# hadleyhzy34/porl

Hardware: AMD Instinct MI355X
Metric: gradient-steps/sec (POR update, batch=1024) (higher is better)
Workload: dtype f32; 1 GPU; POR S=60 A=2 H=1024 L=2 B=1024/GPU (global 1024), 1000000 -row replay (1000000/GPU) resident in HBM, device sampler + gather + full update per step; parallelism=dp1, global_batch=1024

## Files before the change

porl_amd/agent/_iql.py:

```python
from __future__ import annotations

import math
import warnings

import torch
import torch.nn as nn

from ..engine import IqlEngine
from ..parallel import GradExchange



_PIPE_SYNC = __import__("os").environ.get("PORL_PIPE_SYNC", "signal2")
_PIPE_ONECALL = __import__("os").environ.get("PORL_PIPE_ONECALL", "auto")
_DP_POLICY_GROUP = __import__("os").environ.get("PORL_DP_POLICY_GROUP", "1") != "0"
_ONECALL_MAX_WORK = 32 << 20

class ArenaAdam:

    def __init__(self, agent, group, named_params, lr):
        self._agent, self._group = agent, group
        self._names = [n for n, _ in named_params]
        self._params = [p for _, p in named_params]
        self.step_count = 0
# ... 178 lines not shown
                                     wait_policy_seq=max(0, seq - eng.SLOTS) if _PIPE_SYNC == "signal" else 0,
                                     wait_fwd_seq=vr[1] if isinstance(vr, tuple) else 0,
                                     write_policy=_PIPE_SYNC == "signal")
            except Exception:
                eng._seq -= 1
                v_opt.step_count -= 1
                p_opt.step_count -= 1
                raise
            replay.draws += 1
            eng._values_read, eng._policy_done = ("sig", seq), True
            sched.step()
            return self._losses()
        if use_sig:
            main = torch.cuda.current_stream(eng.device)
            eng._seq += 1
            seq = eng._seq
            if _PIPE_SYNC == "signal":
                eng.wait_signal(eng.SIG_POLICY, seq - eng.SLOTS, main)
        elif pipelined:
            eng.wait_slot_free()
        if replay is not None:
            B = eng.load_batch_sampled(replay.rows, batch, replay.seed, replay.draws, replay.act_dim,
                                       self._engine.cfg.weight_mode == 1)
            replay.draws += 1
        else:
            B = eng.load_batch(obs, next_obs, rew, term, pol_target)
        v_opt.step_count += 1
        p_opt.step_count += 1
        hp = self._hyper(B, v_opt, p_opt)
        if not dp and not pipelined:
            eng.step(hp)
            sched.step()
            return self._losses()
        eng.value_backward(hp)
        if dp and self._sharded():
            self._sharded_apply(IqlEngine.GROUP_VF, hp, v_opt)
        else:
            if dp:
                v_opt._unshard()
                ex.allreduce_sum_(eng.grads_vf)
            eng.wait_values_read()
            eng.value_apply(hp)
        if pipelined:
            main, side = torch.cuda.current_stream(eng.device), eng.side_stream()
            k = (v_opt.step_count % eng.SLOTS) * 3
            ev_v, ev_f, ev_p = eng.event(k), eng.event(k + 1), eng.event(k + 2)
            if use_sig:
                eng.signal(eng.SIG_VALUE, seq, main)
            else:
                ev_v.record(main)
            with torch.cuda.stream(side):
                if use_sig:
                    eng.wait_signal(eng.SIG_VALUE, seq, side)
                else:
                    side.wait_event(ev_v)
                eng.policy_forward(hp)
                if use_sig:
                    eng.signal(eng.SIG_FWD, seq, side)
                else:
                    ev_f.record(side)
                eng.policy_backward(hp)
                if dp and self._sharded():
                    self._sharded_apply(IqlEngine.GROUP_POL, hp, p_opt, self._exchange_for(IqlEngine.GROUP_POL, True))
                else:
                    if dp:
                        p_opt._unshard()
# ... 149 lines not shown
```

porl_amd/csrc/porl_api.hip:

```cpp
#include <hip/hip_runtime.h>

#include <algorithm>
#include <cmath>
#include <cstdio>
#include <cstring>
#include <string>
#include <vector>

#include "../../include/porl_hip.h"
#include "gemm_f32.hpp"
#include "gemm_bf16.hpp"
#include "kernels.hpp"
#include "l0_fwd.hpp"
#include "skinny.hpp"
#include "iqn.hpp"
#include "qnet_fused.hpp"
#include "per_tree.hpp"
#include "dist_losses.hpp"
#include "online.hpp"
#include "per_online.hpp"
#include "bcq_mask.hpp"

using namespace porl;

namespace {

thread_local std::string g_err;

#define PORL_FAIL(code, ...)                         \
  do {                                               \
    char _b[512];                                    \
    snprintf(_b, sizeof _b, __VA_ARGS__);            \
    g_err = _b;                                      \
    return (code);                                   \
  } while (0)
// ... 48 lines not shown
} g_prof;

const char* g_phase = "";

struct ProfScope {
  bool active; ProfRec r; hipStream_t s;
  ProfScope(const std::string& label, hipStream_t st, double flops, double bytes) : active(g_prof.on), s(st) {
    if (!active) return;
    r.label = g_prof.label_id(std::string(g_phase) + label); r.flops = flops; r.bytes = bytes;
    r.e0 = g_prof.get(); r.e1 = g_prof.get();
    (void)hipEventRecord(r.e0, s);
  }
  ~ProfScope() {
    if (!active) return;
    (void)hipEventRecord(r.e1, s);
    g_prof.recs.push_back(r);
  }
};

const float* g_dbg_a_scale = nullptr; const float* g_dbg_a_shift = nullptr; const float* g_dbg_resid = nullptr;
float* g_dbg_cstat = nullptr;
unsigned long long* g_qnet_stamps = nullptr;

constexpr int NUM_CU = 256;
constexpr int SK_MAX = 16;
constexpr int NLL_ROWS_PER_BLOCK = 4;
constexpr int LN_ROWS_PER_BLOCK = 8;
constexpr int HEAD_ROWS_PER_BLOCK = HEAD_ROWS;

struct Tune {
  int tile_map[4] = {TILE_64x128, TILE_64x64, TILE_64x128, TILE_64x64};
  int tile_map_short[4] = {TILE_64x64, TILE_64x64, TILE_64x128, TILE_64x64};
  int vbwd_tile_short = -1;
  int l0_kernel = 1;
  int l0_tile = -1;
  int skinny = 7;
  int skinny_pipelined = -1, skinny_pipelined_max_h = 768;
  int dw0_slabs = 16;
  int iql_fold = 1;
  int gemm_lds_pad = 0, gemm_lds_pad_min_blocks = 0;
  int iql_pad_value = 18432, iql_pad_policy = 0, iql_pad_min_blocks = 4 * NUM_CU, iql_pad_min_k = 0;
  int enc_tile_n96 = 0;
  int enc_gemm_sb = 1;
  int enc_patch_rows = 0;
  int enc_s2d = 0;
  int enc_bf16_operands_only = 0;
  int enc_pconv_mfma = 0;
  int enc_bn_sweep = 0;
  int enc_dense_patch = 0;
  int qnet_fused = 1;
  int qnet_rows16 = 1;
  int qnet_wgrad_share = 11;
  int qnet_two_groups = 1;
} g_tune;

enum TuneClamp { TC_ANY, TC_BOOL, TC_NONNEG, TC_1_16, TC_MASK };
struct TuneKey { const char* key; int Tune::*field; TuneClamp clamp; };
#define TK(key, clamp) {#key, &Tune::key, clamp}
const TuneKey k_tune_keys[] = {
    TK(gemm_lds_pad, TC_NONNEG), TK(gemm_lds_pad_min_blocks, TC_NONNEG), TK(iql_pad_value, TC_NONNEG), TK(iql_pad_policy, TC_NONNEG),
    TK(iql_pad_min_blocks, TC_NONNEG), TK(iql_pad_min_k, TC_NONNEG), TK(qnet_fused, TC_BOOL), TK(qnet_two_groups, TC_BOOL),
    TK(qnet_wgrad_share, TC_1_16), TK(qnet_rows16, TC_BOOL), TK(enc_dense_patch, TC_BOOL), TK(enc_s2d, TC_BOOL), TK(enc_patch_rows, TC_NONNEG),
    TK(enc_gemm_sb, TC_ANY), TK(enc_tile_n96, TC_BOOL), TK(enc_bn_sweep, TC_BOOL), TK(enc_pconv_mfma, TC_BOOL), TK(enc_bf16_operands_only, TC_BOOL),
    TK(iql_fold, TC_BOOL), TK(skinny, TC_MASK), TK(skinny_pipelined, TC_MASK), TK(skinny_pipelined_max_h, TC_ANY), TK(dw0_slabs, TC_1_16),
    TK(l0_tile, TC_ANY), TK(l0_kernel, TC_BOOL), TK(vbwd_tile_short, TC_ANY),
};

int tune_apply(Tune& t, const char* key, int value) {
  if (!key) PORL_FAIL(PORL_ERR_INVALID, "null key");
  for (const TuneKey& k : k_tune_keys) {
    if (strcmp(key, k.key)) continue;
    const TuneClamp c = k.clamp;
    t.*k.field = c == TC_BOOL ? value != 0 : c == TC_NONNEG ? std::max(0, value) : c == TC_1_16 ? std::max(1, std::min(value, 16))
               : c == TC_MASK && value == 1 ? 7 : value;
    return PORL_OK;
  }
  const bool sh = !strncmp(key, "tile_map_short", 14);
  const char* i = key + (sh ? 14 : 8);
  if (!strncmp(key, "tile_map", 8) && *i >= '0' && *i <= '3' && !i[1] && value >= 0 && value < TILE_COUNT) {
    (sh ? t.tile_map_short : t.tile_map)[*i - '0'] = value;
    return PORL_OK;
  }
  PORL_FAIL(PORL_ERR_INVALID, "unknown tuning key '%s'", key);
}

inline int64_t ru4(int64_t x) { return (x + 3) & ~int64_t(3); }
inline int cdiv(int a, int b) { return (a + b - 1) / b; }

struct TensorInfo { int64_t off; int rows, cols; };

struct MlpLayout {
  int n_lin = 0;
  int dims[PORL_MAX_HIDDEN + 2] = {0};
  int64_t w[PORL_MAX_HIDDEN + 1] = {0}, b[PORL_MAX_HIDDEN + 1] = {0};
  int64_t lnw[PORL_MAX_HIDDEN] = {0}, lnb[PORL_MAX_HIDDEN] = {0};
  bool ln = false;
};

// ... 28 lines not shown
  int64_t hp_t[2], hp_v[2];
  int64_t act_q[2][2], hp_q[2];
  int64_t dv[2], dmu;
  int64_t slab_mean, slab_a, slab_b, slab_pa;
  int64_t part_loss, part_min, part_dls;
  int64_t xhat_v[2][PORL_MAX_HIDDEN], rstd_v[2][PORL_MAX_HIDDEN];
  int64_t ln_dg[2], ln_db[2], ln_dh[2];
  int64_t head_part[2], head_loss, head_db[2];
  int64_t pol_w;
  int64_t total;
};

}

struct porl_iql {
  porl_iql_cfg cfg;
  MlpLayout v[2], pol;
  int64_t logstd_off = 0, n_vf = 0, n_pol = 0;
  std::vector<TensorInfo> t_vf, t_pol;
  porl_iql_buffers buf{};
  bool bound = false;
  int device = -1;
  int mode = 0;
  int slot = 0;
  ReduceArgs fin_v{}, fin_p{};
  bool fin_v_pending = false, fin_p_pending = false;
  int batch = 0;
  bool have_pol_target = false;
  bool pol_prefetched = false;
  bool pol_fwd_done = false;
  int pol_nslab = 1;
  int Sp = 0, Dp = 0, Hp = 0, parts_max = 0;
  Workspace ws{};
  Tune tune = g_tune;
};

namespace {

int pick_tile(const GemmGroup& g, const Tune& t, bool short_blocks = false) {
  int minM = 1 << 30, minN = 1 << 30, maxK = 0;
  for (int i = 0; i < g.nprob; ++i) {
    minM = std::min(minM, g.p[i].M); minN = std::min(minN, g.p[i].N); maxK = std::max(maxK, g.p[i].K);
  }
  if (maxK <= 128) return TILE_64x64;
  auto blocks = [&](int tile) {
    int bm, bn, n = 0;
    tile_dims(tile, bm, bn);
    for (int i = 0; i < g.nprob; ++i) n += cdiv(g.p[i].M, bm) * cdiv(g.p[i].N, bn) * std::max(1, g.p[i].splitk);
    return n;
  };
  int cand[3], nc = 0;
  if (minN <= 64 && minM <= 64) { cand[nc++] = TILE_64x64; }
  else if (minN <= 64) { cand[nc++] = TILE_128x64; cand[nc++] = TILE_64x64; }
  else if (minM <= 64) { cand[nc++] = TILE_64x128; cand[nc++] = TILE_64x64; }
  else { cand[nc++] = TILE_128x128; cand[nc++] = TILE_128x64; cand[nc++] = TILE_64x64; }
  const int* map = short_blocks ? t.tile_map_short : t.tile_map;
  for (int i = 0; i < nc; ++i)
    if (blocks(cand[i]) >= NUM_CU) return map[cand[i]];
  return map[cand[nc - 1]];
}

int pick_splitk(int M, int N, int K, int nprob, int bm, int bn) {
  const int tiles = nprob * cdiv(M, bm) * cdiv(N, bn);
  int sk = cdiv(NUM_CU, tiles);
  sk = std::min(sk, std::max(1, K / 64));
  return std::max(1, std::min(sk, SK_MAX));
}

int launch_group(GemmGroup& g, int tile, const Tune& t, hipStream_t s, int iql_pad = -1) {
  const bool iql = iql_pad >= 0 && !t.gemm_lds_pad && g.nprob > 0 && g.p[0].K >= t.iql_pad_min_k;
  g.lds_pad = iql ? iql_pad : t.gemm_lds_pad;
  g.lds_pad_min_blocks = iql ? t.iql_pad_min_blocks : t.gemm_lds_pad_min_blocks;
  double flops = 0.0, bytes = 0.0;
  std::string label;
  if (g_prof.on) {
    bool vec = true, apro = false;
    for (int i = 0; i < g.nprob; ++i) {
      const GemmProb& p = g.p[i];
      flops += 2.0 * p.M * p.N * p.K;
      bytes += 4.0 * ((double)p.M * p.K + (double)p.N * p.K + (p.store_c ? (double)p.M * p.N : 0.0));
      vec = vec && p.a_vec && p.b_vec;
      apro = apro || p.apro != APRO_NONE;
    }
    int bm, bn;
    tile_dims(tile, bm, bn);
    const TileCfg tc = tile_cfg(tile);
    label = "gemm_f32_kernel<" + std::to_string(bm) + "," + std::to_string(bn) + "," + std::to_string(GEMM_BK) + "," +
            std::to_string(tc.wm) + "," + std::to_string(tc.wn) + "," + (vec ? "true" : "false") + "," +
            (apro ? "true" : "false") + (g.single_buffer && vec && tile == TILE_64x64 ? ",true>" : ">");
  }
  ProfScope ps(label, s, flops, bytes);
  hipError_t e = launch_gemm_group(tile, g, s);
  if (e != hipSuccess) {
    g_err = std::string("gemm launch: ") + hipGetErrorString(e);
    return (int)e;
  }
  return 0;
}

int launch_group_bf16(GemmGroup& g, int tile, hipStream_t s) {
  double flops = 0.0, bytes = 0.0;
  std::string label;
  if (g_prof.on) {
    for (int i = 0; i < g.nprob; ++i) {
      const GemmProb& p = g.p[i];
// ... 18 lines not shown
  if (r.njobs == 0) return 0;
  long maxn = 0;
  for (int i = 0; i < r.njobs; ++i) maxn = std::max(maxn, r.job[i].n);
  dim3 grid((unsigned)std::min<long>((maxn + 31) / 32, 2048), r.njobs);
  ProfScope ps("multi_reduce_kernel", s, 0.0, 0.0);
  hipLaunchKernelGGL(multi_reduce_kernel, grid, dim3(256), 0, s, r);
  PORL_HIP(hipGetLastError());
  return 0;
}

void add_reduce(ReduceArgs& r, float* out, const float* slab, long n, long stride, int nslab, int op = 0,
                float scale = 1.f) {
  ReduceJob& j = r.job[r.njobs++];
  j.out = out; j.slab = slab; j.bias = nullptr; j.n = n; j.stride = stride; j.nslab = nslab; j.ncols = 1; j.act = 0;
  j.op = op; j.scale = scale; j.adam_off = -1;
  j.width = nslab > 64 ? 4 : 32;
}

int check_ready(const porl_iql* h, bool need_batch) {
  if (!h) PORL_FAIL(PORL_ERR_INVALID, "null engine");
  if (!h->bound) PORL_FAIL(PORL_ERR_UNBOUND, "porl_iql_bind() has not been called");
  if (need_batch && h->batch <= 0) PORL_FAIL(PORL_ERR_INVALID, "no minibatch loaded (porl_iql_load_batch)");
  return 0;
}

bool short_blocks(const porl_iql* h) { return (h->mode & PORL_IQL_MODE_SHORT_BLOCKS) != 0; }
int skinny_mask(const porl_iql* h) {
  const Tune& t = h->tune;
  if (!short_blocks(h)) return t.skinny;
  return t.skinny_pipelined >= 0 ? t.skinny_pipelined : h->cfg.hidden_dim <= t.skinny_pipelined_max_h ? t.skinny : 0;
}
int iql_tile(const porl_iql* h, const GemmGroup& g) { return pick_tile(g, h->tune, short_blocks(h)); }

int iql_launch(const porl_iql* h, GemmGroup& g, int tile, bool policy, hipStream_t s) {
  const Tune& t = h->tune;
  return launch_group(g, tile, t, s, !short_blocks(h) ? -1 : policy ? t.iql_pad_policy : t.iql_pad_value);
}

constexpr int MAX_FWD_NETS = 5;
struct FwdNet {
  const float* in; int ldin;
  const float* W; const float* b;
  float* out;
  const float* headw; float* headout;
  const float* ln_g = nullptr; const float* ln_b = nullptr;
  float* xhat = nullptr; float* rstd = nullptr;
};

int fwd_hidden_layer(porl_iql* h, const FwdNet* nets, int nnets, int B, int K, bool last, int* parts_out, bool policy,
                     hipStream_t s) {
  const int H = h->cfg.hidden_dim;
  if (h->tune.l0_kernel && K <= L0_KP && nnets <= L0_MAX_NETS) {
    L0Args a{};
    a.nnets = nnets; a.B = B; a.H = H; a.K = K; a.ldw = K; a.ldo = h->Hp;
    bool plain = true;
    for (int n = 0; n < nnets; ++n) {
      plain = plain && !nets[n].ln_g && nets[n].out && !(last && nets[n].headw);
      a.net[n] = L0Net{nets[n].in, nets[n].W, nets[n].b, nets[n].out, nets[n].ldin};
    }
    if (plain && l0_fwd_supported(a)) {
      if (parts_out) *parts_out = head_parts(H, 0);
      ProfScope ps("l0_fwd_kernel", s, 2.0 * nnets * B * (double)H * K, 4.0 * nnets * ((double)B * K + (double)H * K + (double)B * H));
      PORL_HIP(launch_l0_fwd(a, s));
      return 0;
    }
  }
  GemmGroup g{};
  g.nprob = nnets;
  bool any_ln = false;
// ... 352 lines not shown
      a.hp_t[i] = W + ws.hp_t[i]; a.hp_v[i] = W + ws.hp_v[i];
      a.b_t[i] = Pt + h->v[i].b[L]; a.b_v[i] = Pv + h->v[i].b[L];
      a.dv[i] = W + ws.dv[i];
      a.db_out[i] = Gv + h->v[i].b[L];
    }
    a.rew = W + ws.rew; a.term = W + ws.term; a.target_v = W + ws.target_v_slot[h->slot]; a.stats = h->buf.stats;
    a.B = B; a.parts = parts; a.tau = hp->tau; a.discount = hp->discount; a.inv_batch = hp->inv_batch;
    hipLaunchKernelGGL(value_loss_kernel, dim3(1), dim3(1024), 0, s, a);
    PORL_HIP(hipGetLastError());
  }

  ReduceArgs red{};
  if (LN) return value_backward_ln(h, hp, s, defer);
  {
    const int nhb = cdiv(B, HEAD_ROWS_PER_BLOCK);
    HeadBwdArgs a{};
    for (int i = 0; i < 2; ++i) {
      a.Hact[i] = W + ws.act_v[i][L - 1]; a.w[i] = Pv + h->v[i].w[L];
      a.dZ[i] = W + ws.dz_v[i][(L - 1) & 1]; a.part_dw[i] = W + ws.head_part[i];
      a.hp_t[i] = W + ws.hp_t[i]; a.hp_v[i] = W + ws.hp_v[i];
      a.b_t[i] = Pt + h->v[i].b[L]; a.b_v[i] = Pv + h->v[i].b[L];
      a.dv[i] = W + ws.dv[i]; a.part_db[i] = W + ws.head_db[i];
      add_reduce(red, Gv + h->v[i].w[L], W + ws.head_part[i], H, H, nhb);
      add_reduce(red, Gv + h->v[i].b[L], W + ws.head_db[i], 1, 1, nhb);
    }
    a.rew = W + ws.rew; a.term = W + ws.term; a.target_v = W + ws.target_v_slot[h->slot]; a.part_loss = W + ws.head_loss;
    add_reduce(red, h->buf.stats, W + ws.head_loss, 1, 1, nhb, 0, hp->inv_batch);
    a.B = B; a.H = H; a.ld = Hp; a.parts = parts;
    a.tau = hp->tau; a.discount = hp->discount; a.inv_batch = hp->inv_batch;
    ProfScope ps("relu_head_bwd_kernel", s, 0.0, 16.0 * B * H);
    hipLaunchKernelGGL(relu_head_bwd_kernel, dim3(nhb, 2), dim3(256), 0, s, a);
    PORL_HIP(hipGetLastError());
  }
  for (int l = L - 1; l >= 0; --l) {
    const int Kin = l == 0 ? S : H;
    if (l == 0) {
      Dw0Net dn[2];
      const int64_t per = (int64_t)H * S, perc = H;
      for (int i = 0; i < 2; ++i) {
        float* slabW = W + ws.slab_a + (int64_t)i * SK_MAX * (per + 2 * perc + 8);
        dn[i] = Dw0Net{W + ws.dz_v[i][0], Gv + h->v[i].w[0], Gv + h->v[i].b[0], slabW, slabW + (int64_t)SK_MAX * per};
      }
      int rc = 0;
      if (dw0_skinny(h, dn, 2, W + ws.xs_slot[h->slot], h->Sp, B, H, S, Hp, red, "V6.dW0:", s, &rc)) {
        if (rc) return rc;
        break;
      }
    }
    GemmGroup g{};
    for (int i = 0; i < 2; ++i) {
      const float* dz = W + ws.dz_v[i][l & 1];
      const float* in = l == 0 ? W + ws.xs_slot[h->slot] : W + ws.act_v[i][l - 1];
      const int ldin = l == 0 ? h->Sp : Hp;
      GemmProb p = make_prob(GEMM_TN, dz, Hp, in, ldin, Gv + h->v[i].w[l], Kin, H, Kin, B);
      p.colsum = Gv + h->v[i].b[l];
      g.p[g.nprob++] = p;
      if (l > 0) {
        GemmProb q = make_prob(GEMM_NN, dz, Hp, Pv + h->v[i].w[l], Kin, W + ws.dz_v[i][(l - 1) & 1], Hp, B, Kin, H);
        q.mask = W + ws.act_v[i][l - 1]; q.ldmask = Hp;
        g.p[g.nprob++] = q;
      }
    }
    int tile = iql_tile(h, g);
    if (l > 0 && short_blocks(h) && h->tune.vbwd_tile_short >= 0) tile = h->tune.vbwd_tile_short;
    if (l == 0) {
      int bm, bn;
      tile_dims(tile, bm, bn);
      const int sk = pick_splitk(H, Kin, B, 2, bm, bn);
      if (sk > 1) {
        const int64_t per = (int64_t)H * Kin, perc = H;
        for (int i = 0; i < 2; ++i) {
          float* slabW = W + ws.slab_a + (int64_t)i * SK_MAX * (per + 2 * perc + 8);
          float* slabC = slabW + (int64_t)SK_MAX * per;
          g.p[i].splitk = sk; g.p[i].C = slabW; g.p[i].colsum = slabC;
          add_reduce(red, Gv + h->v[i].w[0], slabW, per, per, sk);
          add_reduce(red, Gv + h->v[i].b[0], slabC, perc, perc, sk);
        }
      }
    }
    g_phase = l == 0 ? "V6.dW0:" : "V5.bwd:";
    PORL_TRY(iql_launch(h, g, tile, false, s));
  }
  g_phase = "V7.combine:";
  if (defer) *defer = red;
  else PORL_TRY(launch_reduce(red, s));
  g_phase = "";
  return PORL_OK;
}

int porl_iql_value_backward(porl_iql* h, const porl_iql_hyper* hp, void* stream) {
  PORL_TRY(check_ready(h, true)); DevGuard _dg(h->device);
  if (!hp) PORL_FAIL(PORL_ERR_INVALID, "null hyper-parameters");
  const bool fold = (h->mode & PORL_IQL_MODE_FOLD_COMBINE) != 0;
  h->fin_v = ReduceArgs{};
  PORL_TRY(value_backward_impl(h, hp, (hipStream_t)stream, fold ? &h->fin_v : nullptr));
  h->fin_v_pending = fold;
  return PORL_OK;
}

static int adam_launch(float* p, float* g, float* m, float* v, float* tgt, int64_t n, double lr, int step,
                       double b1, double b2, double eps, double ema_beta, hipStream_t s, const ReduceArgs* fin = nullptr) {
  if (n < 0 || n % 4) PORL_FAIL(PORL_ERR_INVALID, "adam range must be a non-negative multiple of 4 floats");
  if (step < 1) PORL_FAIL(PORL_ERR_INVALID, "adam step must be >= 1");
  if (n == 0 && !(fin && fin->njobs)) return PORL_OK;
  AdamArgs a{};
  a.p = p; a.g = g; a.m = m; a.v = v; a.tgt = tgt;
  const double bc1 = 1.0 - std::pow(b1, (double)step);
  const double bc2 = 1.0 - std::pow(b2, (double)step);
  a.s.step_size = (float)(lr / bc1);
  a.s.bc2_sqrt = (float)std::sqrt(bc2);
  a.s.omb1 = (float)(1.0 - b1); a.s.beta2 = (float)b2; a.s.omb2 = (float)(1.0 - b2);
  a.s.eps = (float)eps; a.s.ema_beta = (float)ema_beta; a.s.omeb = (float)(1.0 - ema_beta);
  a.n4 = n / 4;
  const int sweep_blocks = (int)std::min<long>((a.n4 + 255) / 256, 1 << 20);
  a.span4 = sweep_blocks ? ((a.n4 + sweep_blocks - 1) / sweep_blocks + 255) / 256 * 256 : 256;
  int reduce_blocks = 0;
  double extra_bytes = 0.0;
  if (fin) {
    for (int q = 0; q < fin->njobs; ++q) {
      ReduceJob j = fin->job[q];
      const bool inside = j.out >= g && j.out + j.n <= g + n;
      const long off = inside ? (long)(j.out - g) : -1;
      extra_bytes += 4.0 * (double)j.n * j.nslab;
      const bool plain = j.op == 0 && j.scale == 1.f && !j.bias && j.act == 0;
      if (inside && plain && j.nslab <= ADAM_SWEEP_SLABS && off % 4 == 0 && j.n % 4 == 0 && j.stride % 4 == 0 &&
          aligned16(j.slab) && a.nregions < MAX_ADAM_REGIONS) {
        AdamRegion& R = a.region[a.nregions++];
        R.lo = off; R.hi = off + j.n; R.slab = j.slab; R.stride = j.stride; R.nslab = j.nslab;
// ... 220 lines not shown
    a.tiles_n = cdiv(H, SKN_T);
    skn_split(cdiv(B, SKN_T), SK_MAX, a.nslab, a.rtiles);
    a.slabW_stride = (long)D * H; a.slabC_stride = D;
    add_reduce(red, Gp + h->pol.w[L], a.slabW, (long)D * H, (long)D * H, a.nslab);
    add_reduce(red, Gp + h->pol.b[L], a.slabC, D, D, a.nslab);
    g_phase = "P5.outbwd:";
    {
      ProfScope ps("out_bwd_kernel", s, 4.0 * B * (double)H * D, 4.0 * (2.0 * B * H + (double)B * D + (double)D * H + (double)a.nslab * D * H));
      hipLaunchKernelGGL(out_bwd_kernel, dim3(a.nslab * a.tiles_n), dim3(256), 0, s, a);
    }
    g_phase = "";
    PORL_HIP(hipGetLastError());
  } else {
    GemmGroup g{};
    g.nprob = 2;
    g.p[0] = make_prob(GEMM_TN, W + ws.dmu, Dp, W + ws.act_p[L - 1], Hp, Gp + h->pol.w[L], H, D, H, B);
    g.p[0].colsum = Gp + h->pol.b[L];
    g.p[1] = make_prob(GEMM_NN, W + ws.dmu, Dp, Pp + h->pol.w[L], H, W + ws.dz_p[(L - 1) & 1], Hp, B, H, D);
    g.p[1].mask = W + ws.act_p[L - 1]; g.p[1].ldmask = Hp;
    const int tile = D <= 64 ? TILE_64x128 : iql_tile(h, g);
    int bm, bn;
    tile_dims(tile, bm, bn);
    const int sk = pick_splitk(D, H, B, 1, bm, bn);
    if (sk > 1) {
      float* slabW = W + ws.slab_b;
      float* slabC = slabW + (int64_t)SK_MAX * D * H;
      g.p[0].splitk = sk; g.p[0].C = slabW; g.p[0].colsum = slabC;
      add_reduce(red, Gp + h->pol.w[L], slabW, (long)D * H, (long)D * H, sk);
      add_reduce(red, Gp + h->pol.b[L], slabC, D, D, sk);
    }
    g_phase = "P5.outbwd:";
    PORL_TRY(iql_launch(h, g, tile, true, s));
  }
  for (int l = L - 1; l >= 0; --l) {
    const int Kin = l == 0 ? S : H;
    if (l == 0) {
      const int64_t per = (int64_t)H * S;
      float* slabW = W + ws.slab_pa;
      Dw0Net dn{W + ws.dz_p[0], Gp + h->pol.w[0], Gp + h->pol.b[0], slabW, slabW + (int64_t)SK_MAX * per};
      int rc = 0;
      if (dw0_skinny(h, &dn, 1, W + ws.xs_slot[h->slot], h->Sp, B, H, S, Hp, red, "P7.dW0:", s, &rc)) {
        if (rc) return rc;
        break;
      }
    }
    const float* dz = W + ws.dz_p[l & 1];
    const float* in = l == 0 ? W + ws.xs_slot[h->slot] : W + ws.act_p[l - 1];
    const int ldin = l == 0 ? h->Sp : Hp;
    GemmGroup g{};
    g.p[g.nprob] = make_prob(GEMM_TN, dz, Hp, in, ldin, Gp + h->pol.w[l], Kin, H, Kin, B);
    g.p[g.nprob++].colsum = Gp + h->pol.b[l];
    if (l > 0) {
      GemmProb q = make_prob(GEMM_NN, dz, Hp, Pp + h->pol.w[l], Kin, W + ws.dz_p[(l - 1) & 1], Hp, B, Kin, H);
      q.mask = W + ws.act_p[l - 1]; q.ldmask = Hp;
      g.p[g.nprob++] = q;
    }
    const int tile = iql_tile(h, g);
    if (l == 0) {
      int bm, bn;
      tile_dims(tile, bm, bn);
      const int sk = pick_splitk(H, Kin, B, 1, bm, bn);
      if (sk > 1) {
        const int64_t per = (int64_t)H * Kin;
        float* slabW = W + ws.slab_pa;
        float* slabC = slabW + (int64_t)SK_MAX * per;
        g.p[0].splitk = sk; g.p[0].C = slabW; g.p[0].colsum = slabC;
        add_reduce(red, Gp + h->pol.w[0], slabW, per, per, sk);
        add_reduce(red, Gp + h->pol.b[0], slabC, H, H, sk);
      }
    }
    g_phase = l == 0 ? "P7.dW0:" : "P6.bwd:";
    PORL_TRY(iql_launch(h, g, tile, true, s));
  }
  g_phase = "P8.combine:";
  if (defer) *defer = red;
  else PORL_TRY(launch_reduce(red, s));
  g_phase = "";
  return PORL_OK;
}

int porl_iql_policy_forward(porl_iql* h, const porl_iql_hyper* hp, void* stream) {
  PORL_TRY(check_ready(h, true)); DevGuard _dg(h->device);
  if (!hp) PORL_FAIL(PORL_ERR_INVALID, "null hyper-parameters");
  return policy_backward_impl(h, hp, (hipStream_t)stream, nullptr, 1);
}

int porl_iql_policy_backward(porl_iql* h, const porl_iql_hyper* hp, void* stream) {
  PORL_TRY(check_ready(h, true)); DevGuard _dg(h->device);
  if (!hp) PORL_FAIL(PORL_ERR_INVALID, "null hyper-parameters");
  const bool fold = (h->mode & PORL_IQL_MODE_FOLD_COMBINE) != 0;
  h->fin_p = ReduceArgs{};
  PORL_TRY(policy_backward_impl(h, hp, (hipStream_t)stream, fold ? &h->fin_p : nullptr));
  h->fin_p_pending = fold;
  return PORL_OK;
}

int porl_iql_step(porl_iql* h, const porl_iql_hyper* hp, void* stream) {
  PORL_TRY(check_ready(h, true)); DevGuard _dg(h->device);
  if (!hp) PORL_FAIL(PORL_ERR_INVALID, "null hyper-parameters");
  hipStream_t s = (hipStream_t)stream;
  ReduceArgs fin{};
  PORL_TRY(value_backward_impl(h, hp, s, h->tune.iql_fold ? &fin : nullptr));
  g_phase = "V8.";
  PORL_TRY(adam_launch(h->buf.params_vf, h->buf.grads_vf, h->buf.adam_m_vf, h->buf.adam_v_vf, h->buf.params_tgt, h->n_vf,
                       hp->value_lr, hp->value_step, hp->adam_beta1, hp->adam_beta2, hp->adam_eps, hp->ema_beta, s, &fin));
  fin = ReduceArgs{};
// ... 385 lines not shown
  PORL_HIP(hipGetLastError());
  return PORL_OK;
}

int porl_per_sample_slots(const double* tree, int64_t capacity, const double* u, int32_t batch, int64_t n_entries,
                          double beta, int64_t* out_idx, int64_t* out_slots, float* out_w, float* out_wmean,
                          double* scratch, void* stream) {
  if (!tree || !u || !out_idx || !out_slots || !out_w || !out_wmean || !scratch) PORL_FAIL(PORL_ERR_INVALID, "null argument");
  if (capacity < 1 || batch < 1 || n_entries < 1 || n_entries > capacity)
    PORL_FAIL(PORL_ERR_INVALID, "need capacity >= 1, batch >= 1, 1 <= n_entries <= capacity");
  DevGuard _dg(device_of(tree));
  PerSampleSlotsArgs a{tree, capacity, u, batch, n_entries, beta, out_idx, out_slots, out_w, out_wmean, scratch};
  hipLaunchKernelGGL(per_sample_slots_kernel, dim3(1), dim3(256), 0, (hipStream_t)stream, a);
  PORL_HIP(hipGetLastError());
  return PORL_OK;
}

int porl_per_update_f32(double* tree, int64_t capacity, const int64_t* tree_idx, const float* td_abs, int32_t n, double eps,
                        double alpha, int32_t* stamp, void* stream) {
  if (!tree || !tree_idx || !td_abs || !stamp) PORL_FAIL(PORL_ERR_INVALID, "null argument");
  if (capacity < 1 || n < 1) PORL_FAIL(PORL_ERR_INVALID, "need capacity >= 1 and n >= 1");
  DevGuard _dg(device_of(tree));
  const int threads = n >= 1024 ? 1024 : (n + 63) / 64 * 64;
  hipLaunchKernelGGL(per_update_f32_kernel, dim3(1), dim3(threads), 0, (hipStream_t)stream, tree, tree_idx, td_abs, n, capacity,
                     eps, alpha, stamp, per_levels(capacity));
  PORL_HIP(hipGetLastError());
  return PORL_OK;
}

int porl_tune_set(const char* key, int value) { return tune_apply(g_tune, key, value); }

int porl_iql_tune_set(porl_iql* h, const char* key, int value) {
  if (!h) PORL_FAIL(PORL_ERR_INVALID, "null engine");
  return tune_apply(h->tune, key, value);
}

int porl_signal_create(void** out) {
  if (!out) PORL_FAIL(PORL_ERR_INVALID, "null argument");
  int dev = 0, can = 0;
  PORL_HIP(hipGetDevice(&dev));
  PORL_HIP(hipDeviceGetAttribute(&can, hipDeviceAttributeCanUseStreamWaitValue, dev));
  if (!can) PORL_FAIL(PORL_ERR_UNSUPPORTED, "stream wait-value operations are not supported on this device");
  void* p = nullptr;
  PORL_HIP(hipExtMallocWithFlags(&p, 8, hipMallocSignalMemory));
  PORL_HIP(hipMemset(p, 0, 8));
  *out = p;
  return PORL_OK;
}
int porl_signal_destroy(void* sig) {
  if (sig) PORL_HIP(hipFree(sig));
  return PORL_OK;
}
int porl_signal_write(void* sig, uint64_t value, void* stream) {
  if (!sig) PORL_FAIL(PORL_ERR_INVALID, "null signal");
  PORL_HIP(hipStreamWriteValue64((hipStream_t)stream, sig, value, 0));
  return PORL_OK;
}
int porl_signal_wait_ge(void* sig, uint64_t value, void* stream) {
  if (!sig) PORL_FAIL(PORL_ERR_INVALID, "null signal");
  PORL_HIP(hipStreamWaitValue64((hipStream_t)stream, sig, value, hipStreamWaitValueGte, 0xFFFFFFFFFFFFFFFFull));
  return PORL_OK;
}

int porl_iql_update_pipelined(porl_iql* h, const porl_iql_hyper* hp, int32_t batch, const float* rows, int64_t row_stride,
                              int64_t n_rows, int32_t act_dim, int32_t target_is_action, uint64_t seed, uint64_t step,
                              void* sig_value, void* sig_fwd, void* sig_policy, uint64_t seq, uint64_t wait_policy_seq,
                              uint64_t wait_fwd_seq, int32_t write_policy, void* main_stream, void* side_stream) {
  PORL_TRY(check_ready(h, false)); DevGuard _dg(h->device);
  if (!hp) PORL_FAIL(PORL_ERR_INVALID, "null hyper-parameters");
  if (!sig_value || !sig_fwd || !sig_policy || seq < 1) PORL_FAIL(PORL_ERR_INVALID, "three signal counters and seq >= 1 are required");
  if (main_stream == side_stream) PORL_FAIL(PORL_ERR_INVALID, "the two phases need two streams");
  if (!(h->mode & PORL_IQL_MODE_TWO_SLOTS) || !(h->mode & PORL_IQL_MODE_FOLD_COMBINE))
    PORL_FAIL(PORL_ERR_INVALID, "pipelined updates need PORL_IQL_MODE_TWO_SLOTS | PORL_IQL_MODE_FOLD_COMBINE");
  if (batch < 1 || batch > h->cfg.max_batch) PORL_FAIL(PORL_ERR_INVALID, "batch %d outside [1,%d]", batch, h->cfg.max_batch);
  if (!rows || n_rows < batch || n_rows > (int64_t(1) << 40) || act_dim < 0 ||
      row_stride < 2 * (int64_t)h->cfg.obs_dim + 2 + act_dim)
    PORL_FAIL(PORL_ERR_INVALID, "bad replay rows (need batch <= n_rows <= 2^40, row stride >= 2*S+2+A)");
  if (target_is_action ? h->cfg.pol_out_dim != act_dim : h->cfg.pol_out_dim != h->cfg.obs_dim)
    PORL_FAIL(PORL_ERR_INVALID, "policy target width mismatch");
  if (wait_policy_seq) PORL_TRY(porl_signal_wait_ge(sig_policy, wait_policy_seq, main_stream));
  PORL_TRY(porl_iql_load_batch_sampled(h, batch, rows, row_stride, n_rows, act_dim, target_is_action, seed, step, nullptr, main_stream));
  PORL_TRY(porl_iql_value_backward(h, hp, main_stream));
  if (wait_fwd_seq) PORL_TRY(porl_signal_wait_ge(sig_fwd, wait_fwd_seq, main_stream));
  PORL_TRY(porl_iql_value_apply(h, hp, main_stream));
  PORL_TRY(porl_signal_write(sig_value, seq, main_stream));
  PORL_TRY(porl_signal_wait_ge(sig_value, seq, side_stream));
  PORL_TRY(porl_iql_policy_forward(h, hp, side_stream));
  PORL_TRY(porl_signal_write(sig_fwd, seq, side_stream));
  PORL_TRY(porl_iql_policy_backward(h, hp, side_stream));
  PORL_TRY(porl_iql_policy_apply(h, hp, side_stream));
  if (write_policy) PORL_TRY(porl_signal_write(sig_policy, seq, side_stream));
  return PORL_OK;
}

int porl_tune_set_ptr(const char* key, void* ptr) {
  if (!key) PORL_FAIL(PORL_ERR_INVALID, "null key");
  if (!strcmp(key, "qnet_stamps")) { g_qnet_stamps = (unsigned long long*)ptr; return PORL_OK; }
  if (!strcmp(key, "gemm_a_scale")) { g_dbg_a_scale = (const float*)ptr; return PORL_OK; }
  if (!strcmp(key, "gemm_a_shift")) { g_dbg_a_shift = (const float*)ptr; return PORL_OK; }
  if (!strcmp(key, "gemm_resid")) { g_dbg_resid = (const float*)ptr; return PORL_OK; }
  if (!strcmp(key, "gemm_cstat")) { g_dbg_cstat = (float*)ptr; return PORL_OK; }
  PORL_FAIL(PORL_ERR_INVALID, "unknown tuning key '%s'", key);
}

int porl_state2costmap(float* state, int64_t state_rs, int32_t batch, int32_t n_ang, int32_t n_dist, float* out,
                        void* stream) {
  if (!state || !out || batch < 1 || n_ang < 4 || n_dist < 4) PORL_FAIL(PORL_ERR_INVALID, "bad costmap arguments");
  if (batch > 65535) PORL_FAIL(PORL_ERR_INVALID, "batch > 65535");
  DevGuard _dg(device_of(out));
  hipStream_t s = (hipStream_t)stream;
  const double pi = 3.14159265358979323846;
  const float dist_inc = (float)((4.0 + 1e-4) / n_dist);
  const float ang_inc = (float)((2.0 * pi + 1e-4) / n_ang);
  const float deg_min = (float)(-pi + (2.0 * pi + 2e-4) / n_ang), deg_max = (float)(pi - (2.0 * pi + 2e-4) / n_ang);
  const float dist_max = (float)(4.0 - 4.0 / n_dist);
  hipLaunchKernelGGL(costmap_kernel, dim3(n_ang, batch), dim3(std::min(256, n_dist)), 0, s, state, (long)state_rs, n_ang,
// ... 1052 lines not shown
```

porl_amd/engine.py:

```python
from __future__ import annotations

import ctypes as C
import math

import numpy as np
import torch

from . import _native as N


def _norm_device(device):
    device = torch.device(device)
    if device.type == "cuda" and device.index is None:
        device = torch.device("cuda", torch.cuda.current_device())
    return device


class IqlEngine:
    GROUP_VF, GROUP_POL = 0, 1
    MODE_TWO_SLOTS, MODE_FOLD_COMBINE, MODE_SHORT_BLOCKS = 1, 2, 4
    SLOTS = 3

    def __init__(self, obs_dim, pol_out_dim, hidden_dim, n_hidden, layer_norm=False, pol_tanh=False,
                 weight_mode=0, max_batch=1024, device="cpu"):
# ... 40 lines not shown
                    sig.append(p)
            self._signals = sig
            self._seq = 0
        return self._signals or None

    def signal(self, which, value, stream):
        N.check(self._lib.porl_signal_write(self.signals()[which], int(value), C.c_void_p(stream.cuda_stream)), "porl_signal_write")

    def wait_signal(self, which, value, stream):
        if value > 0:
            N.check(self._lib.porl_signal_wait_ge(self.signals()[which], int(value), C.c_void_p(stream.cuda_stream)),
                    "porl_signal_wait_ge")

    def join(self):
        ev, self._policy_done, self._values_read = self._policy_done, None, None
        self._slot_users = [None] * self.SLOTS
        if ev is True:
            ev = self.event(3 * self.SLOTS)
            ev.record(self.side_stream())
        if ev is not None:
            torch.cuda.current_stream(self.device).wait_event(ev)

    def wait_slot_free(self):
        ev = self._slot_users[0]
        if ev is not None:
            torch.cuda.current_stream(self.device).wait_event(ev)

    def wait_values_read(self):
        ev, self._values_read = self._values_read, None
        if isinstance(ev, tuple):
            self.wait_signal(self.SIG_FWD, ev[1], torch.cuda.current_stream(self.device))
        elif ev is not None:
            torch.cuda.current_stream(self.device).wait_event(ev)

    def set_mode(self, mode):
        if mode != self._mode:
            N.check(self._lib.porl_iql_set_mode(self._h, int(mode)), "porl_iql_set_mode")
            self._mode = mode

    def tune_set(self, key, value):
        N.check(self._lib.porl_iql_tune_set(self._h, key.encode(), int(value)), "porl_iql_tune_set")

    SLICE_QUANTUM = 4 * 840

    def _alloc(self):
        dev = self.device
        q = self.SLICE_QUANTUM
        z = lambda n: torch.zeros((n + q - 1) // q * q, dtype=torch.float32, device=dev)
        self.params_vf, self.params_tgt, self.params_pol = z(self.n_vf), z(self.n_vf), z(self.n_pol)
        self.grads_vf, self.grads_pol = z(self.n_vf), z(self.n_pol)
        self.adam_m_vf, self.adam_v_vf = z(self.n_vf), z(self.n_vf)
        self.adam_m_pol, self.adam_v_pol = z(self.n_pol), z(self.n_pol)
        self.stats = z(8)
        self.workspace = None
        self._bound = False

    def _ensure_bound(self):
        if self.device.type != "cuda":
            raise N.NativeError("porl_amd computes on a HIP device only (device='cuda'); there is no CPU path")
        if self._bound:
            return
        nws = int(self._lib.porl_iql_workspace_floats(self._h))
        self.workspace = torch.empty(nws, dtype=torch.float32, device=self.device)
        b = N.IqlBuffers(*[C.c_void_p(t.data_ptr()) for t in (
            self.params_vf, self.params_tgt, self.params_pol, self.grads_vf, self.grads_pol,
            self.adam_m_vf, self.adam_v_vf, self.adam_m_pol, self.adam_v_pol, self.workspace, self.stats)])
# ... 149 lines not shown
                                                  N.current_stream_ptr(self.device)), "porl_iql_forward_policy")
        return mean

    SMALL_BATCH = 8

    def forward_policy_host(self, x):
        self._ensure_bound()
        self.join()
        B, D, S = int(x.shape[0]), self.cfg.pol_out_dim, self.cfg.obs_dim
        if B < 1 or B > self.SMALL_BATCH or tuple(x.shape) != (B, S):
            raise RuntimeError(f"obs: expected shape (1..{self.SMALL_BATCH}, {S}), got {tuple(x.shape)}")
        if getattr(self, "_pin", None) is None:
            self._pin = (torch.empty(self.SMALL_BATCH, S, dtype=torch.float32).pin_memory(),
                         torch.empty(self.SMALL_BATCH, D, dtype=torch.float32).pin_memory())
        pin_in, pin_out = self._pin
        if isinstance(x, torch.Tensor) and x.device.type == "cuda":
            if x.dtype != torch.float32:
                raise RuntimeError(f"obs: expected float32, got {x.dtype}")
            src = x if x.stride(1) == 1 else x.contiguous()
            xp, xrs = N.ptr(src), src.stride(0)
        else:
            pin_in[:B].copy_(torch.as_tensor(x, dtype=torch.float32))
            xp, xrs = N.ptr(pin_in), S
        stream = torch.cuda.current_stream(self.device)
        N.check(self._lib.porl_iql_forward_policy(self._h, xp, xrs, B, N.ptr(pin_out), D, C.c_void_p(stream.cuda_stream)),
                "porl_iql_forward_policy")
        stream.synchronize()
        return pin_out[:B].numpy().copy()

    def _free_signals(self):
        for p in (getattr(self, "_signals", None) or []):
            self._lib.porl_signal_destroy(p)
        self._signals = None

    def __del__(self):
        try:
            self._free_signals()
            if getattr(self, "_h", None):
                self._lib.porl_iql_destroy(self._h)
                self._h = None
        except Exception:
            pass


class IqnEngine:

    MAX_EMBED, MAX_TAU, MAX_ACTIONS, ACT_MAX_INLINE = 128, 256, 64, 256

    def __init__(self, state_dim, n_actions, embedding_dim, hidden, max_batch, max_tau, device):
        self.device = _norm_device(device)
        S, A, Ed, H = int(state_dim), int(n_actions), int(embedding_dim), int(hidden)
        numel = [H * S, H, H * H, H, H * Ed, H, H * H, H, A * H, A]
        offs, off = [], 0
        for k in numel:
            offs.append(off)
            off += (k + 3) // 4 * 4
        self.offsets, self.n_params = offs, off
        self.cfg = N.IqnCfg(S, A, Ed, H, int(max_batch), int(max_tau), (C.c_int64 * 10)(*offs), off)
        self._lib = N.lib()
        h = C.c_void_p()
        N.check(self._lib.porl_iqn_create(C.byref(self.cfg), C.byref(h)), "porl_iqn_create")
        self._h = h
        self.stats = self.workspace = None
        self._bound = False

    def bind(self, params, params_tgt, grads, adam_m, adam_v):
# ... 137 lines not shown
```

Measured before the change: 3057 gradient-steps/sec.

## Split hidden-layer backward GEMMs and move the side-stream value wait inside value backward

Value and policy backward can now split each hidden layer's grouped GEMM into a dz (input-gradient) launch and a weight-gradient launch, with the layer-0 dW GEMM placed between them, so the dependent chain moves forward sooner. This is gated by tuning flags that default to off. The cross-stream wait on the forward-read signal is no longer issued after value_backward. It is armed and issued inside value_backward, either at the end or, when vwait_early is set, just before dW0. The goal is to let backward work overlap with the side-stream policy forward that reads the values. The cost is more launches and a more complex signal handshake, passed through tune_set.

```diff
diff --git a/porl_amd/agent/_iql.py b/porl_amd/agent/_iql.py
--- a/porl_amd/agent/_iql.py
+++ b/porl_amd/agent/_iql.py
@@ -234,6 +234,8 @@
             eng.step(hp)
             sched.step()
             return self._losses()
+        if use_sig and not dp:
+            eng.arm_values_read_wait()
         eng.value_backward(hp)
         if dp and self._sharded():
             self._sharded_apply(IqlEngine.GROUP_VF, hp, v_opt)
diff --git a/porl_amd/csrc/porl_api.hip b/porl_amd/csrc/porl_api.hip
--- a/porl_amd/csrc/porl_api.hip
+++ b/porl_amd/csrc/porl_api.hip
@@ -1,6 +1,7 @@
 #include <hip/hip_runtime.h>
 
 #include <algorithm>
+#include <climits>
 #include <cmath>
 #include <cstdio>
 #include <cstring>
@@ -115,6 +116,7 @@
   int tile_map[4] = {TILE_64x128, TILE_64x64, TILE_64x128, TILE_64x64};
   int tile_map_short[4] = {TILE_64x64, TILE_64x64, TILE_64x128, TILE_64x64};
   int vbwd_tile_short = -1;
+  int vbwd_split = 0, vwait_early = 0, pbwd_split = 0, split_pad = 1;
   int l0_kernel = 1;
   int l0_tile = -1;
   int skinny = 7;
@@ -147,6 +149,7 @@
     TK(enc_gemm_sb, TC_ANY), TK(enc_tile_n96, TC_BOOL), TK(enc_bn_sweep, TC_BOOL), TK(enc_pconv_mfma, TC_BOOL), TK(enc_bf16_operands_only, TC_BOOL),
     TK(iql_fold, TC_BOOL), TK(skinny, TC_MASK), TK(skinny_pipelined, TC_MASK), TK(skinny_pipelined_max_h, TC_ANY), TK(dw0_slabs, TC_1_16),
     TK(l0_tile, TC_ANY), TK(l0_kernel, TC_BOOL), TK(vbwd_tile_short, TC_ANY),
+    TK(vbwd_split, TC_BOOL), TK(vwait_early, TC_BOOL), TK(pbwd_split, TC_BOOL), TK(split_pad, TC_BOOL),
 };
 
 int tune_apply(Tune& t, const char* key, int value) {
@@ -241,6 +244,9 @@
   int pol_nslab = 1;
   int Sp = 0, Dp = 0, Hp = 0, parts_max = 0;
   Workspace ws{};
+  void* vwait_sig = nullptr;
+  uint64_t vwait_seq = 0, vwait_seq_hi = 0;
+  bool vwait_armed = false;
   Tune tune = g_tune;
 };
 
@@ -276,10 +282,11 @@
   return std::max(1, std::min(sk, SK_MAX));
 }
 
-int launch_group(GemmGroup& g, int tile, const Tune& t, hipStream_t s, int iql_pad = -1) {
+int launch_group(GemmGroup& g, int tile, const Tune& t, hipStream_t s, int iql_pad = -1, int judge_blocks = -1) {
   const bool iql = iql_pad >= 0 && !t.gemm_lds_pad && g.nprob > 0 && g.p[0].K >= t.iql_pad_min_k;
   g.lds_pad = iql ? iql_pad : t.gemm_lds_pad;
   g.lds_pad_min_blocks = iql ? t.iql_pad_min_blocks : t.gemm_lds_pad_min_blocks;
+  if (judge_blocks >= 0) g.lds_pad_min_blocks = judge_blocks >= g.lds_pad_min_blocks ? 0 : INT_MAX;
   double flops = 0.0, bytes = 0.0;
   std::string label;
   if (g_prof.on) {
@@ -364,9 +371,16 @@
 }
 int iql_tile(const porl_iql* h, const GemmGroup& g) { return pick_tile(g, h->tune, short_blocks(h)); }
 
-int iql_launch(const porl_iql* h, GemmGroup& g, int tile, bool policy, hipStream_t s) {
+int iql_launch(const porl_iql* h, GemmGroup& g, int tile, bool policy, hipStream_t s, int judge_blocks = -1) {
   const Tune& t = h->tune;
-  return launch_group(g, tile, t, s, !short_blocks(h) ? -1 : policy ? t.iql_pad_policy : t.iql_pad_value);
+  return launch_group(g, tile, t, s, !short_blocks(h) ? -1 : policy ? t.iql_pad_policy : t.iql_pad_value, judge_blocks);
+}
+
+int issue_vwait(porl_iql* h, hipStream_t s) {
+  if (!h->vwait_armed) return 0;
+  h->vwait_armed = false;
+  PORL_HIP(hipStreamWaitValue64(s, h->vwait_sig, h->vwait_seq, hipStreamWaitValueGte, 0xFFFFFFFFFFFFFFFFull));
+  return 0;
 }
 
 constexpr int MAX_FWD_NETS = 5;
@@ -785,9 +799,10 @@
     hipLaunchKernelGGL(relu_head_bwd_kernel, dim3(nhb, 2), dim3(256), 0, s, a);
     PORL_HIP(hipGetLastError());
   }
-  for (int l = L - 1; l >= 0; --l) {
-    const int Kin = l == 0 ? S : H;
-    if (l == 0) {
+  const bool split = short_blocks(h) && h->tune.vbwd_split;
+  auto dw0 = [&]() -> int {
+    if (short_blocks(h) && h->tune.vwait_early) PORL_TRY(issue_vwait(h, s));
+    {
       Dw0Net dn[2];
       const int64_t per = (int64_t)H * S, perc = H;
       for (int i = 0; i < 2; ++i) {
@@ -795,45 +810,60 @@
         dn[i] = Dw0Net{W + ws.dz_v[i][0], Gv + h->v[i].w[0], Gv + h->v[i].b[0], slabW, slabW + (int64_t)SK_MAX * per};
       }
       int rc = 0;
-      if (dw0_skinny(h, dn, 2, W + ws.xs_slot[h->slot], h->Sp, B, H, S, Hp, red, "V6.dW0:", s, &rc)) {
-        if (rc) return rc;
-        break;
-      }
+      if (dw0_skinny(h, dn, 2, W + ws.xs_slot[h->slot], h->Sp, B, H, S, Hp, red, "V6.dW0:", s, &rc)) return rc;
     }
     GemmGroup g{};
     for (int i = 0; i < 2; ++i) {
+      GemmProb p = make_prob(GEMM_TN, W + ws.dz_v[i][0], Hp, W + ws.xs_slot[h->slot], h->Sp, Gv + h->v[i].w[0], S, H, S, B);
+      p.colsum = Gv + h->v[i].b[0];
+      g.p[g.nprob++] = p;
+    }
+    const int tile = iql_tile(h, g);
+    int bm, bn;
+    tile_dims(tile, bm, bn);
+    const int sk = pick_splitk(H, S, B, 2, bm, bn);
+    if (sk > 1) {
+      const int64_t per = (int64_t)H * S, perc = H;
+      for (int i = 0; i < 2; ++i) {
+        float* slabW = W + ws.slab_a + (int64_t)i * SK_MAX * (per + 2 * perc + 8);
+        float* slabC = slabW + (int64_t)SK_MAX * per;
+        g.p[i].splitk = sk; g.p[i].C = slabW; g.p[i].colsum = slabC;
+        add_reduce(red, Gv + h->v[i].w[0], slabW, per, per, sk);
+        add_reduce(red, Gv + h->v[i].b[0], slabC, perc, perc, sk);
+      }
+    }
+    g_phase = "V6.dW0:";
+    return iql_launch(h, g, tile, false, s);
+  };
+  bool dw0_done = false;
+  for (int l = L - 1; l > 0; --l) {
+    GemmGroup g{}, gz{}, gw{};
+    for (int i = 0; i < 2; ++i) {
       const float* dz = W + ws.dz_v[i][l & 1];
-      const float* in = l == 0 ? W + ws.xs_slot[h->slot] : W + ws.act_v[i][l - 1];
-      const int ldin = l == 0 ? h->Sp : Hp;
-      GemmProb p = make_prob(GEMM_TN, dz, Hp, in, ldin, Gv + h->v[i].w[l], Kin, H, Kin, B);
+      GemmProb p = make_prob(GEMM_TN, dz, Hp, W + ws.act_v[i][l - 1], Hp, Gv + h->v[i].w[l], H, H, H, B);
       p.colsum = Gv + h->v[i].b[l];
-      g.p[g.nprob++] = p;
-      if (l > 0) {
-        GemmProb q = make_prob(GEMM_NN, dz, Hp, Pv + h->v[i].w[l], Kin, W + ws.dz_v[i][(l - 1) & 1], Hp, B, Kin, H);
-        q.mask = W + ws.act_v[i][l - 1]; q.ldmask = Hp;
-        g.p[g.nprob++] = q;
-      }
+      GemmProb q = make_prob(GEMM_NN, dz, Hp, Pv + h->v[i].w[l], H, W + ws.dz_v[i][(l - 1) & 1], Hp, B, H, H);
+      q.mask = W + ws.act_v[i][l - 1]; q.ldmask = Hp;
+      g.p[g.nprob++] = p; g.p[g.nprob++] = q;
+      gw.p[gw.nprob++] = p; gz.p[gz.nprob++] = q;
     }
     int tile = iql_tile(h, g);
-    if (l > 0 && short_blocks(h) && h->tune.vbwd_tile_short >= 0) tile = h->tune.vbwd_tile_short;
-    if (l == 0) {
-      int bm, bn;
-      tile_dims(tile, bm, bn);
-      const int sk = pick_splitk(H, Kin, B, 2, bm, bn);
-      if (sk > 1) {
-        const int64_t per = (int64_t)H * Kin, perc = H;
-        for (int i = 0; i < 2; ++i) {
-          float* slabW = W + ws.slab_a + (int64_t)i * SK_MAX * (per + 2 * perc + 8);
-          float* slabC = slabW + (int64_t)SK_MAX * per;
-          g.p[i].splitk = sk; g.p[i].C = slabW; g.p[i].colsum = slabC;
-          add_reduce(red, Gv + h->v[i].w[0], slabW, per, per, sk);
-          add_reduce(red, Gv + h->v[i].b[0], slabC, perc, perc, sk);
-        }
-      }
-    }
-    g_phase = l == 0 ? "V6.dW0:" : "V5.bwd:";
-    PORL_TRY(iql_launch(h, g, tile, false, s));
-  }
+    if (short_blocks(h) && h->tune.vbwd_tile_short >= 0) tile = h->tune.vbwd_tile_short;
+    g_phase = "V5.bwd:";
+    if (!split) {
+      PORL_TRY(iql_launch(h, g, tile, false, s));
+      continue;
+    }
+    const int joint = h->tune.split_pad ? plan_group(g, tile) : -1;
+    PORL_TRY(iql_launch(h, gz, tile, false, s, joint));
+    if (l == 1) {
+      PORL_TRY(dw0());
+      dw0_done = true;
+      g_phase = "V5.bwd:";
+    }
+    PORL_TRY(iql_launch(h, gw, tile, false, s, joint));
+  }
+  if (!dw0_done) PORL_TRY(dw0());
   g_phase = "V7.combine:";
   if (defer) *defer = red;
   else PORL_TRY(launch_reduce(red, s));
@@ -842,11 +872,16 @@
 }
 
 int porl_iql_value_backward(porl_iql* h, const porl_iql_hyper* hp, void* stream) {
+  struct Disarm {
+    porl_iql* h;
+    ~Disarm() { if (h) h->vwait_armed = false; }
+  } _disarm{h};
   PORL_TRY(check_ready(h, true)); DevGuard _dg(h->device);
   if (!hp) PORL_FAIL(PORL_ERR_INVALID, "null hyper-parameters");
   const bool fold = (h->mode & PORL_IQL_MODE_FOLD_COMBINE) != 0;
   h->fin_v = ReduceArgs{};
   PORL_TRY(value_backward_impl(h, hp, (hipStream_t)stream, fold ? &h->fin_v : nullptr));
+  PORL_TRY(issue_vwait(h, (hipStream_t)stream));
   h->fin_v_pending = fold;
   return PORL_OK;
 }
@@ -1133,46 +1168,55 @@
     g_phase = "P5.outbwd:";
     PORL_TRY(iql_launch(h, g, tile, true, s));
   }
-  for (int l = L - 1; l >= 0; --l) {
-    const int Kin = l == 0 ? S : H;
-    if (l == 0) {
-      const int64_t per = (int64_t)H * S;
-      float* slabW = W + ws.slab_pa;
-      Dw0Net dn{W + ws.dz_p[0], Gp + h->pol.w[0], Gp + h->pol.b[0], slabW, slabW + (int64_t)SK_MAX * per};
-      int rc = 0;
-      if (dw0_skinny(h, &dn, 1, W + ws.xs_slot[h->slot], h->Sp, B, H, S, Hp, red, "P7.dW0:", s, &rc)) {
-        if (rc) return rc;
-        break;
-      }
-    }
+  const bool split = short_blocks(h) && h->tune.pbwd_split;
+  auto dw0 = [&]() -> int {
+    const int64_t per = (int64_t)H * S;
+    float* slabW = W + ws.slab_pa;
+    float* slabC = slabW + (int64_t)SK_MAX * per;
+    Dw0Net dn{W + ws.dz_p[0], Gp + h->pol.w[0], Gp + h->pol.b[0], slabW, slabC};
+    int rc = 0;
+    if (dw0_skinny(h, &dn, 1, W + ws.xs_slot[h->slot], h->Sp, B, H, S, Hp, red, "P7.dW0:", s, &rc)) return rc;
+    GemmGroup g{};
+    g.p[g.nprob] = make_prob(GEMM_TN, W + ws.dz_p[0], Hp, W + ws.xs_slot[h->slot], h->Sp, Gp + h->pol.w[0], S, H, S, B);
+    g.p[g.nprob++].colsum = Gp + h->pol.b[0];
+    const int tile = iql_tile(h, g);
+    int bm, bn;
+    tile_dims(tile, bm, bn);
+    const int sk = pick_splitk(H, S, B, 1, bm, bn);
+    if (sk > 1) {
+      g.p[0].splitk = sk; g.p[0].C = slabW; g.p[0].colsum = slabC;
+      add_reduce(red, Gp + h->pol.w[0], slabW, per, per, sk);
+      add_reduce(red, Gp + h->pol.b[0], slabC, H, H, sk);
+    }
+    g_phase = "P7.dW0:";
+    return iql_launch(h, g, tile, true, s);
+  };
+  bool dw0_done = false;
+  for (int l = L - 1; l > 0; --l) {
     const float* dz = W + ws.dz_p[l & 1];
-    const float* in = l == 0 ? W + ws.xs_slot[h->slot] : W + ws.act_p[l - 1];
-    const int ldin = l == 0 ? h->Sp : Hp;
-    GemmGroup g{};
-    g.p[g.nprob] = make_prob(GEMM_TN, dz, Hp, in, ldin, Gp + h->pol.w[l], Kin, H, Kin, B);
+    GemmGroup g{}, gz{}, gw{};
+    g.p[g.nprob] = make_prob(GEMM_TN, dz, Hp, W + ws.act_p[l - 1], Hp, Gp + h->pol.w[l], H, H, H, B);
     g.p[g.nprob++].colsum = Gp + h->pol.b[l];
-    if (l > 0) {
-      GemmProb q = make_prob(GEMM_NN, dz, Hp, Pp + h->pol.w[l], Kin, W + ws.dz_p[(l - 1) & 1], Hp, B, Kin, H);
-      q.mask = W + ws.act_p[l - 1]; q.ldmask = Hp;
-      g.p[g.nprob++] = q;
-    }
+    GemmProb q = make_prob(GEMM_NN, dz, Hp, Pp + h->pol.w[l], H, W + ws.dz_p[(l - 1) & 1], Hp, B, H, H);
+    q.mask = W + ws.act_p[l - 1]; q.ldmask = Hp;
+    g.p[g.nprob++] = q;
+    gw.p[gw.nprob++] = g.p[0]; gz.p[gz.nprob++] = q;
     const int tile = iql_tile(h, g);
-    if (l == 0) {
-      int bm, bn;
-      tile_dims(tile, bm, bn);
-      const int sk = pick_splitk(H, Kin, B, 1, bm, bn);
-      if (sk > 1) {
-        const int64_t per = (int64_t)H * Kin;
-        float* slabW = W + ws.slab_pa;
-        float* slabC = slabW + (int64_t)SK_MAX * per;
-        g.p[0].splitk = sk; g.p[0].C = slabW; g.p[0].colsum = slabC;
-        add_reduce(red, Gp + h->pol.w[0], slabW, per, per, sk);
-        add_reduce(red, Gp + h->pol.b[0], slabC, H, H, sk);
-      }
-    }
-    g_phase = l == 0 ? "P7.dW0:" : "P6.bwd:";
-    PORL_TRY(iql_launch(h, g, tile, true, s));
-  }
+    g_phase = "P6.bwd:";
+    if (!split) {
+      PORL_TRY(iql_launch(h, g, tile, true, s));
+      continue;
+    }
+    const int joint = h->tune.split_pad ? plan_group(g, tile) : -1;
+    PORL_TRY(iql_launch(h, gz, tile, true, s, joint));
+    if (l == 1) {
+      PORL_TRY(dw0());
+      dw0_done = true;
+      g_phase = "P6.bwd:";
+    }
+    PORL_TRY(iql_launch(h, gw, tile, true, s, joint));
+  }
+  if (!dw0_done) PORL_TRY(dw0());
   g_phase = "P8.combine:";
   if (defer) *defer = red;
   else PORL_TRY(launch_reduce(red, s));
@@ -1624,6 +1668,19 @@
 
 int porl_iql_tune_set(porl_iql* h, const char* key, int value) {
   if (!h) PORL_FAIL(PORL_ERR_INVALID, "null engine");
+  if (key && !strncmp(key, "vwait_s", 7)) {
+    const uint64_t v = (uint32_t)value;
+    uint64_t sig = (uint64_t)(uintptr_t)h->vwait_sig;
+    if (!strcmp(key, "vwait_sig_lo")) { h->vwait_sig = (void*)(uintptr_t)((sig & ~0xFFFFFFFFull) | v); return PORL_OK; }
+    if (!strcmp(key, "vwait_sig_hi")) { h->vwait_sig = (void*)(uintptr_t)((sig & 0xFFFFFFFFull) | (v << 32)); return PORL_OK; }
+    if (!strcmp(key, "vwait_seq_hi")) { h->vwait_seq_hi = v; return PORL_OK; }
+    if (!strcmp(key, "vwait_seq")) {
+      if (!h->vwait_sig) PORL_FAIL(PORL_ERR_INVALID, "vwait_seq needs the counter's address first (vwait_sig_lo / _hi)");
+      h->vwait_seq = (h->vwait_seq_hi << 32) | v;
+      h->vwait_armed = true;
+      return PORL_OK;
+    }
+  }
   return tune_apply(h->tune, key, value);
 }
 
@@ -1672,8 +1729,8 @@
     PORL_FAIL(PORL_ERR_INVALID, "policy target width mismatch");
   if (wait_policy_seq) PORL_TRY(porl_signal_wait_ge(sig_policy, wait_policy_seq, main_stream));
   PORL_TRY(porl_iql_load_batch_sampled(h, batch, rows, row_stride, n_rows, act_dim, target_is_action, seed, step, nullptr, main_stream));
+  if (wait_fwd_seq) { h->vwait_sig = sig_fwd; h->vwait_seq = wait_fwd_seq; h->vwait_armed = true; }
   PORL_TRY(porl_iql_value_backward(h, hp, main_stream));
-  if (wait_fwd_seq) PORL_TRY(porl_signal_wait_ge(sig_fwd, wait_fwd_seq, main_stream));
   PORL_TRY(porl_iql_value_apply(h, hp, main_stream));
   PORL_TRY(porl_signal_write(sig_value, seq, main_stream));
   PORL_TRY(porl_signal_wait_ge(sig_value, seq, side_stream));
diff --git a/porl_amd/engine.py b/porl_amd/engine.py
--- a/porl_amd/engine.py
+++ b/porl_amd/engine.py
@@ -96,6 +96,23 @@
             self.wait_signal(self.SIG_FWD, ev[1], torch.cuda.current_stream(self.device))
         elif ev is not None:
             torch.cuda.current_stream(self.device).wait_event(ev)
+
+    def arm_values_read_wait(self):
+        ev = self._values_read
+        if not isinstance(ev, tuple):
+            return False
+        self._values_read = None
+        i32 = lambda v: v - (1 << 32) if v >= 1 << 31 else v
+        addr, seq = int(self.signals()[self.SIG_FWD].value), int(ev[1])
+        sent = getattr(self, "_vwait_sent", None)
+        if sent is None or sent[0] != addr:
+            self.tune_set("vwait_sig_lo", i32(addr & 0xFFFFFFFF))
+            self.tune_set("vwait_sig_hi", i32(addr >> 32))
+        if sent is None or sent[1] != seq >> 32:
+            self.tune_set("vwait_seq_hi", i32(seq >> 32))
+        self._vwait_sent = (addr, seq >> 32)
+        self.tune_set("vwait_seq", i32(seq & 0xFFFFFFFF))
+        return True
 
     def set_mode(self, mode):
         if mode != self._mode:
@@ -311,6 +328,7 @@
         for p in (getattr(self, "_signals", None) or []):
             self._lib.porl_signal_destroy(p)
         self._signals = None
+        self._vwait_sent = None
 
     def __del__(self):
         try:
```

Measured after the change: 3031 gradient-steps/sec (median of 2 runs). About the same (-0.8%).
